# nianticlabs/mickey

Measured on AMD Instinct MI355X. Metric: image pairs/sec (540x720), higher is better.
Workload: dtype bf16

## Files before the change

### mickey_amd/csrc/mk_attention.hip

```cpp
#include <type_traits>

#include "mk_common.hpp"

namespace mk {
void launch_attn_f32(const float* q, const float* k, const float* vt, float* out, int ldo, int nimg, int heads, int ntok,
                     int ntok_pad, hipStream_t st);
}

namespace {
using namespace mk;

constexpr int KV_TILE_BYTES = 64 * 64 * 2;
constexpr float ATT_REBASE_SUM = 4096.0f;

struct AttnBlock {
  int qblk, head, img;
};
__device__ __forceinline__ AttnBlock attn_block() {
  const int lin = blockIdx.x + gridDim.x * (blockIdx.y + gridDim.y * blockIdx.z);
  const int r = xcd_remap(lin, gridDim.x * gridDim.y * gridDim.z);
  const int hg = r / gridDim.x;
  return AttnBlock{r - hg * (int)gridDim.x, hg % (int)gridDim.y, hg / (int)gridDim.y};
}

template <typename T, int QB>
__global__ __launch_bounds__(256, 2) void attn_fwd_kernel(const T* __restrict__ q, const T* __restrict__ k,
                                                          const T* __restrict__ vt, T* __restrict__ out, int ldo, int heads,
                                                          int ntok, int ntok_pad) {
  using V8 = typename Lp<T>::V8;
  using V4 = typename Lp<T>::V4;
  __shared__ __attribute__((aligned(16))) char smem[4 * KV_TILE_BYTES];

  const int lane = threadIdx.x & 63;
  const int wave = __builtin_amdgcn_readfirstlane(threadIdx.x >> 6);
  const AttnBlock ab = attn_block();
  const int head = ab.head, img = ab.img;
  const long long hb = (long long)img * heads + head;
  const T* Qh = q + hb * ntok_pad * 64;
  const T* Kh = k + hb * ntok_pad * 64;
  const T* Vh = vt + hb * 64 * ntok_pad;
  const int q0 = ab.qblk * (128 * QB) + wave * (32 * QB);
  const int j = lane & 31, hi = lane >> 5;
  const bool wave_has_queries = q0 < ntok;

  V8 qf[QB][4];
#pragma unroll
  for (int qb = 0; qb < QB; ++qb) {
    int qrow = q0 + qb * 32 + j;
    qrow = qrow < ntok_pad ? qrow : ntok_pad - 1;
#pragma unroll
    for (int ks = 0; ks < 4; ++ks) qf[qb][ks] = *(const V8*)(Qh + (long long)qrow * 64 + ks * 16 + hi * 8);
  }

  const int srow = lane >> 3, sp = lane & 7;
  auto stage = [&](int buf, int kt) {
    char* sK = smem + buf * 2 * KV_TILE_BYTES;
    char* sV = sK + KV_TILE_BYTES;
#pragma unroll
    for (int t = 0; t < 2; ++t) {
      const int ii = wave * 2 + t;
      const int r = ii * 8 + srow;
      glds16(Kh + (long long)(kt * 64 + r) * 64 + swz8(r, sp) * 8, sK + ii * 1024);
      glds16(Vh + (long long)r * ntok_pad + kt * 64 + swz8(r, sp) * 8, sV + ii * 1024);
    }
  };

  f32x16 o[QB][2];
  float m_run[QB], l_run[QB];
#pragma unroll
  for (int qb = 0; qb < QB; ++qb) {
#pragma unroll
    for (int i = 0; i < 16; ++i) o[qb][0][i] = o[qb][1][i] = 0.f;
    m_run[qb] = -1e30f;
    l_run[qb] = 0.f;
  }

  const int nkt = (ntok + 63) >> 6;
  stage(0, 0);
  auto kv_tile = [&](const int kt, auto last_tag) {
    constexpr bool LAST = decltype(last_tag)::value;
    asm volatile("s_waitcnt vmcnt(0)" ::: "memory");
    __syncthreads();
    if (!LAST) stage((kt + 1) & 1, kt + 1);
    if (!wave_has_queries) return;
    const char* sK = smem + (kt & 1) * 2 * KV_TILE_BYTES;
    const char* sV = sK + KV_TILE_BYTES;

    f32x16 s[QB][2];
#pragma unroll
    for (int kb = 0; kb < 2; ++kb) {
#pragma unroll
      for (int qb = 0; qb < QB; ++qb)
#pragma unroll
        for (int i = 0; i < 16; ++i) s[qb][kb][i] = 0.f;
      const int row = kb * 32 + j;
#pragma unroll
      for (int ks = 0; ks < 4; ++ks) {
        const V8 kf = *(const V8*)(sK + row * 128 + swz8(row, ks * 2 + hi) * 16);
#pragma unroll
        for (int qb = 0; qb < QB; ++qb) s[qb][kb] = Lp<T>::mma32(kf, qf[qb][ks], s[qb][kb]);
      }
    }
    V8 pf[QB][4];
#pragma unroll
    for (int qb = 0; qb < QB; ++qb) {
      if (LAST && (ntok & 63)) {
#pragma unroll
        for (int kb = 0; kb < 2; ++kb)
#pragma unroll
          for (int r = 0; r < 16; ++r) {
            const int key = kt * 64 + kb * 32 + (r & 3) + 8 * (r >> 2) + 4 * hi;
            if (key >= ntok) s[qb][kb][r] = -1e30f;
          }
      }
      float t8[8];
#pragma unroll
      for (int r = 0; r < 8; ++r)
        t8[r] = fmaxf(fmaxf(s[qb][0][r], s[qb][0][r + 8]), fmaxf(s[qb][1][r], s[qb][1][r + 8]));
      float mx = fmaxf(fmaxf(fmaxf(t8[0], t8[1]), t8[2]), fmaxf(fmaxf(t8[3], t8[4]), t8[5]));
      mx = fmaxf(fmaxf(mx, t8[6]), t8[7]);
      mx = fmaxf(mx, __shfl_xor(mx, 32, 64));
      const float m_new = fmaxf(m_run[qb], mx);
      const bool grew = m_new > m_run[qb];
      float rs4[4] = {0.f, 0.f, 0.f, 0.f};
#pragma unroll
      for (int kb = 0; kb < 2; ++kb)
#pragma unroll
        for (int r = 0; r < 16; ++r) {
          const float pv = __builtin_amdgcn_exp2f(s[qb][kb][r] - m_new);
          s[qb][kb][r] = pv;
          rs4[r & 3] += pv;
        }
      const float rs = (rs4[0] + rs4[1]) + (rs4[2] + rs4[3]);
      if (__any(grew)) {
        const float alpha = __builtin_amdgcn_exp2f(m_run[qb] - m_new);
        l_run[qb] *= alpha;
#pragma unroll
        for (int i = 0; i < 16; ++i) {
          o[qb][0][i] *= alpha;
          o[qb][1][i] *= alpha;
        }
      }
      m_run[qb] = m_new;
      l_run[qb] += rs;
#pragma unroll
      for (int s4 = 0; s4 < 4; ++s4)
#pragma unroll
        for (int e = 0; e < 8; ++e) pf[qb][s4][e] = (T)s[qb][s4 >> 1][(s4 & 1) * 8 + e];
    }
#pragma unroll
    for (int dt = 0; dt < 2; ++dt) {
      const int row = dt * 32 + j;
#pragma unroll
      for (int s4 = 0; s4 < 4; ++s4) {
        const V8 vf = *(const V8*)(sV + row * 128 + swz8(row, s4 * 2 + hi) * 16);
#pragma unroll
        for (int qb = 0; qb < QB; ++qb) o[qb][dt] = Lp<T>::mma32(vf, pf[qb][s4], o[qb][dt]);
      }
    }
  };
  for (int kt = 0; kt < nkt - 1; ++kt) kv_tile(kt, std::false_type{});
  kv_tile(nkt - 1, std::true_type{});

#pragma unroll
  for (int qb = 0; qb < QB; ++qb) {
    const float l_tot = l_run[qb] + __shfl_xor(l_run[qb], 32, 64);
    const float inv = 1.0f / l_tot;
    const int qi = q0 + qb * 32 + j;
    if (qi < ntok) {
      T* orow = out + ((long long)img * ntok + qi) * ldo + head * 64;
#pragma unroll
      for (int dt = 0; dt < 2; ++dt)
#pragma unroll
        for (int r4 = 0; r4 < 4; ++r4) {
          V4 w;
#pragma unroll
          for (int e = 0; e < 4; ++e) w[e] = (T)(o[qb][dt][r4 * 4 + e] * inv);
          *(V4*)(orow + dt * 32 + r4 * 8 + hi * 4) = w;
        }
    }
  }
}

template <typename T, int QB>
__device__ __forceinline__ void attn_fold_wave(const T* __restrict__ Qh, const T* __restrict__ Kh, const T* __restrict__ Vh,
                                               T* __restrict__ out, int ldo, int img, int head, int ntok, int ntok_pad, char* smem,
                                               int lane, int wave, int q0) {
  using V8 = typename Lp<T>::V8;
  using V4 = typename Lp<T>::V4;
  const int j = lane & 31, hi = lane >> 5;
  const bool wave_has_queries = q0 < ntok;

  V8 qf[QB][4];
#pragma unroll
  for (int qb = 0; qb < QB; ++qb) {
    int qrow = q0 + qb * 32 + j;
    qrow = qrow < ntok_pad ? qrow : ntok_pad - 1;
#pragma unroll
    for (int ks = 0; ks < 4; ++ks) qf[qb][ks] = *(const V8*)(Qh + (long long)qrow * 64 + ks * 16 + hi * 8);
  }
  const int srow = lane >> 3, sp = lane & 7;
  auto stage = [&](int buf, int kt) {
    char* sK = smem + buf * 2 * KV_TILE_BYTES;
    char* sV = sK + KV_TILE_BYTES;
#pragma unroll
    for (int t = 0; t < 2; ++t) {
      const int ii = wave * 2 + t;
      const int r = ii * 8 + srow;
      glds16(Kh + (long long)(kt * 64 + r) * 64 + swz8(r, sp) * 8, sK + ii * 1024);
      glds16(Vh + (long long)r * ntok_pad + kt * 64 + swz8(r, sp) * 8, sV + ii * 1024);
    }
  };

  f32x16 o[QB][2], negm[QB];
  float m_run[QB], l_run[QB];
#pragma unroll
  for (int qb = 0; qb < QB; ++qb) {
#pragma unroll
    for (int i = 0; i < 16; ++i) {
      o[qb][0][i] = o[qb][1][i] = 0.f;
      negm[qb][i] = 0.f;
    }
    m_run[qb] = l_run[qb] = 0.f;
  }
  bool first = true;

  const int nkt = (ntok + 63) >> 6;
  stage(0, 0);
  auto kv_tile = [&](const int kt, auto last_tag) {
    constexpr bool LAST = decltype(last_tag)::value;
    asm volatile("s_waitcnt vmcnt(0)" ::: "memory");
    __syncthreads();
    if (!LAST) stage((kt + 1) & 1, kt + 1);
    if (!wave_has_queries) return;
    const char* sK = smem + (kt & 1) * 2 * KV_TILE_BYTES;
    const char* sV = sK + KV_TILE_BYTES;

    f32x16 s[QB][2];
    const bool half_tile = LAST && (ntok & 63) != 0 && (ntok & 63) <= 32;
#pragma unroll
    for (int kb = 0; kb < 2; ++kb) {
      if (LAST && kb == 1 && half_tile) {
#pragma unroll
        for (int qb = 0; qb < QB; ++qb)
#pragma unroll
          for (int r = 0; r < 16; ++r) s[qb][1][r] = -1e30f;
        continue;
      }
      const int row = kb * 32 + j;
#pragma unroll
      for (int ks = 0; ks < 4; ++ks) {
        const V8 kf = *(const V8*)(sK + row * 128 + swz8(row, ks * 2 + hi) * 16);
#pragma unroll
        for (int qb = 0; qb < QB; ++qb) s[qb][kb] = Lp<T>::mma32(kf, qf[qb][ks], ks == 0 ? negm[qb] : s[qb][kb]);
      }
    }
    V8 pf[QB][4];
#pragma unroll
    for (int qb = 0; qb < QB; ++qb) {
      if (LAST && (ntok & 63)) {
#pragma unroll
        for (int kb = 0; kb < 2; ++kb)
#pragma unroll
          for (int r = 0; r < 16; ++r) {
            const int key = kt * 64 + kb * 32 + (r & 3) + 8 * (r >> 2) + 4 * hi;
            if (key >= ntok) s[qb][kb][r] = -1e30f;
          }
      }
      auto exp_sum = [&]() {
        float rs4[4] = {0.f, 0.f, 0.f, 0.f};
#pragma unroll
        for (int s4 = 0; s4 < 4; ++s4)
#pragma unroll
          for (int e = 0; e < 8; ++e) {
            const float pv = __builtin_amdgcn_exp2f(s[qb][s4 >> 1][(s4 & 1) * 8 + e]);
            pf[qb][s4][e] = (T)pv;
            rs4[e & 3] += pv;
          }
        return (rs4[0] + rs4[1]) + (rs4[2] + rs4[3]);
      };
      float rs = 0.f;
      bool rebase = first;
      if (!first) {
        rs = exp_sum();
        rebase = __any(!(rs <= ATT_REBASE_SUM));
      }
      if (rebase) {
        float t8[8];
#pragma unroll
        for (int r = 0; r < 8; ++r) t8[r] = fmaxf(fmaxf(s[qb][0][r], s[qb][0][r + 8]), fmaxf(s[qb][1][r], s[qb][1][r + 8]));
        float mx = fmaxf(fmaxf(fmaxf(t8[0], t8[1]), t8[2]), fmaxf(fmaxf(t8[3], t8[4]), t8[5]));
        mx = fmaxf(fmaxf(mx, t8[6]), t8[7]);
        mx = fmaxf(mx, __shfl_xor(mx, 32, 64));
        const float shift = first ? mx : fmaxf(mx, 0.f);
        const float alpha = first ? 1.0f : __builtin_amdgcn_exp2f(-shift);
#pragma unroll
        for (int i = 0; i < 16; ++i) {
          o[qb][0][i] *= alpha;
          o[qb][1][i] *= alpha;
          s[qb][0][i] -= shift;
          s[qb][1][i] -= shift;
        }
        l_run[qb] *= alpha;
        m_run[qb] += shift;
#pragma unroll
        for (int i = 0; i < 16; ++i) negm[qb][i] = -m_run[qb];
        rs = exp_sum();
      }
      l_run[qb] += rs;
    }
    first = false;
#pragma unroll
    for (int dt = 0; dt < 2; ++dt) {
      const int row = dt * 32 + j;
#pragma unroll
      for (int s4 = 0; s4 < 4; ++s4) {
        if (LAST && s4 >= 2 && half_tile) break;
        const V8 vf = *(const V8*)(sV + row * 128 + swz8(row, s4 * 2 + hi) * 16);
#pragma unroll
        for (int qb = 0; qb < QB; ++qb) o[qb][dt] = Lp<T>::mma32(vf, pf[qb][s4], o[qb][dt]);
      }
    }
  };
  for (int kt = 0; kt < nkt - 1; ++kt) kv_tile(kt, std::false_type{});
  kv_tile(nkt - 1, std::true_type{});

#pragma unroll
  for (int qb = 0; qb < QB; ++qb) {
    const float inv = 1.0f / (l_run[qb] + __shfl_xor(l_run[qb], 32, 64));
    const int qi = q0 + qb * 32 + j;
    if (qi < ntok) {
      T* orow = out + ((long long)img * ntok + qi) * ldo + head * 64;
#pragma unroll
      for (int dt = 0; dt < 2; ++dt)
#pragma unroll
        for (int r4 = 0; r4 < 4; ++r4) {
          V4 w;
#pragma unroll
          for (int e = 0; e < 4; ++e) w[e] = (T)(o[qb][dt][r4 * 4 + e] * inv);
          *(V4*)(orow + dt * 32 + r4 * 8 + hi * 4) = w;
        }
    }
  }
}

template <typename T, int QB, bool TAIL1 = true>
__global__ __launch_bounds__(256, QB == 2 ? 2 : 3) void attn_fwd_fold_kernel(const T* __restrict__ q, const T* __restrict__ k,
                                                                              const T* __restrict__ vt, T* __restrict__ out,
                                                                              int ldo, int heads, int ntok, int ntok_pad) {
  __shared__ __attribute__((aligned(16))) char smem[4 * KV_TILE_BYTES];
  const int lane = threadIdx.x & 63;
  const int wave = __builtin_amdgcn_readfirstlane(threadIdx.x >> 6);
  const AttnBlock ab = attn_block();
  const int head = ab.head, img = ab.img;
  const long long hb = (long long)img * heads + head;
  const T* Qh = q + hb * ntok_pad * 64;
  const T* Kh = k + hb * ntok_pad * 64;
  const T* Vh = vt + hb * 64 * ntok_pad;
  const int q0 = ab.qblk * (128 * QB) + wave * (32 * QB);
  if constexpr (QB == 2 && TAIL1) {
    if (q0 < ntok && q0 + 32 >= ntok) {
      attn_fold_wave<T, 1>(Qh, Kh, Vh, out, ldo, img, head, ntok, ntok_pad, smem, lane, wave, q0);
      return;
    }
  }
  attn_fold_wave<T, QB>(Qh, Kh, Vh, out, ldo, img, head, ntok, ntok_pad, smem, lane, wave, q0);
}

template <typename T, int QB>
__global__ __launch_bounds__(256, QB == 2 ? 2 : 3) void attn_fwd_fold16_kernel(const T* __restrict__ q, const T* __restrict__ k,
                                                                                const T* __restrict__ vt, T* __restrict__ out,
                                                                                int ldo, int heads, int ntok, int ntok_pad) {
  using V8 = typename Lp<T>::V8;
  using V4 = typename Lp<T>::V4;
  __shared__ __attribute__((aligned(16))) char smem[4 * KV_TILE_BYTES];

  const int lane = threadIdx.x & 63;
  const int wave = __builtin_amdgcn_readfirstlane(threadIdx.x >> 6);
  const AttnBlock ab = attn_block();
  const int head = ab.head, img = ab.img;
  const long long hb = (long long)img * heads + head;
  const T* Qh = q + hb * ntok_pad * 64;
  const T* Kh = k + hb * ntok_pad * 64;
  const T* Vh = vt + hb * 64 * ntok_pad;
  const int q0 = ab.qblk * (128 * QB) + wave * (32 * QB);
  const int n = lane & 15, g = lane >> 4;
  const bool wave_has_queries = q0 < ntok;

  V8 qf[QB][2][2];
#pragma unroll
  for (int qb = 0; qb < QB; ++qb)
#pragma unroll
    for (int nb = 0; nb < 2; ++nb) {
      int qrow = q0 + qb * 32 + nb * 16 + n;
      qrow = qrow < ntok_pad ? qrow : ntok_pad - 1;
#pragma unroll
      for (int ks = 0; ks < 2; ++ks) qf[qb][nb][ks] = *(const V8*)(Qh + (long long)qrow * 64 + ks * 32 + g * 8);
    }
  const int srow = lane >> 3, sp = lane & 7;
  auto stage = [&](int buf, int kt) {
    char* sK = smem + buf * 2 * KV_TILE_BYTES;
    char* sV = sK + KV_TILE_BYTES;
#pragma unroll
    for (int t = 0; t < 2; ++t) {
      const int ii = wave * 2 + t;
      const int r = ii * 8 + srow;
      glds16(Kh + (long long)(kt * 64 + r) * 64 + swz8(r, sp) * 8, sK + ii * 1024);
      glds16(Vh + (long long)r * ntok_pad + kt * 64 + swz8(r, sp) * 8, sV + ii * 1024);
    }
  };

  f32x4 o[QB][2][4], negm[QB][2];
  float m_run[QB][2], l_run[QB][2];
#pragma unroll
  for (int qb = 0; qb < QB; ++qb)
#pragma unroll
    for (int nb = 0; nb < 2; ++nb) {
#pragma unroll
      for (int db = 0; db < 4; ++db) o[qb][nb][db] = f32x4{0.f, 0.f, 0.f, 0.f};
      negm[qb][nb] = f32x4{0.f, 0.f, 0.f, 0.f};
      m_run[qb][nb] = l_run[qb][nb] = 0.f;
    }
  bool first = true;
  const int pq = ((g & 1) << 1) | (g >> 1);

  const int nkt = (ntok + 63) >> 6;
  stage(0, 0);
  auto kv_tile = [&](const int kt, auto last_tag) {
    constexpr bool LAST = decltype(last_tag)::value;
    asm volatile("s_waitcnt vmcnt(0)" ::: "memory");
    __syncthreads();
    if (!LAST) stage((kt + 1) & 1, kt + 1);
    if (!wave_has_queries) return;
    const char* sK = smem + (kt & 1) * 2 * KV_TILE_BYTES;
    const char* sV = sK + KV_TILE_BYTES;

    f32x4 s[QB][2][4];
#pragma unroll
    for (int ks = 0; ks < 2; ++ks) {
#pragma unroll
      for (int kb = 0; kb < 4; ++kb) {
        const int row = kb * 16 + n;
        const V8 kf = *(const V8*)(sK + row * 128 + swz8(row, ks * 4 + g) * 16);
#pragma unroll
        for (int qb = 0; qb < QB; ++qb)
#pragma unroll
          for (int nb = 0; nb < 2; ++nb)
            s[qb][nb][kb] = Lp<T>::mma16(kf, qf[qb][nb][ks], ks == 0 ? negm[qb][nb] : s[qb][nb][kb]);
      }
    }
    V8 pf[QB][2][2];
#pragma unroll
    for (int qb = 0; qb < QB; ++qb)
#pragma unroll
      for (int nb = 0; nb < 2; ++nb) {
        if (LAST && (ntok & 63)) {
#pragma unroll
          for (int kb = 0; kb < 4; ++kb)
#pragma unroll
            for (int r = 0; r < 4; ++r)
              if (kt * 64 + kb * 16 + 4 * g + r >= ntok) s[qb][nb][kb][r] = -1e30f;
        }
        auto exp_sum = [&]() {
          float rs4[4] = {0.f, 0.f, 0.f, 0.f};
#pragma unroll
          for (int kb = 0; kb < 4; ++kb)
#pragma unroll
            for (int r = 0; r < 4; ++r) {
              const float pv = __builtin_amdgcn_exp2f(s[qb][nb][kb][r]);
              pf[qb][nb][kb >> 1][(kb & 1) * 4 + r] = (T)pv;
              rs4[r] += pv;
            }
          return (rs4[0] + rs4[1]) + (rs4[2] + rs4[3]);
        };
        float rs = 0.f;
        bool rebase = first;
        if (!first) {
          rs = exp_sum();
          rebase = __any(!(rs <= ATT_REBASE_SUM));
        }
        if (rebase) {
          float t4[4];
#pragma unroll
          for (int r = 0; r < 4; ++r) t4[r] = fmaxf(fmaxf(s[qb][nb][0][r], s[qb][nb][1][r]), fmaxf(s[qb][nb][2][r], s[qb][nb][3][r]));
          float mx = fmaxf(fmaxf(t4[0], t4[1]), fmaxf(t4[2], t4[3]));
          mx = fmaxf(mx, __shfl_xor(mx, 16, 64));
          mx = fmaxf(mx, __shfl_xor(mx, 32, 64));
          const float shift = first ? mx : fmaxf(mx, 0.f);
          const float alpha = first ? 1.0f : __builtin_amdgcn_exp2f(-shift);
#pragma unroll
          for (int b4 = 0; b4 < 4; ++b4)
#pragma unroll
            for (int i = 0; i < 4; ++i) {
              o[qb][nb][b4][i] *= alpha;
              s[qb][nb][b4][i] -= shift;
// ... 108 lines not shown
```

### mickey_amd/csrc/mk_gemm_common.hpp

```cpp
#pragma once
#include "mk_common.hpp"

namespace mk {
namespace gemm {

constexpr int BK = 64;
template <typename T> constexpr int EPC = 16 / (int)sizeof(T);
template <typename T> constexpr int KT = 128 / (int)sizeof(T);

enum AMode { A_DENSE = 0, A_CONV3 = 1 };

struct GemmParams {
  const void* A;
  const void* A2;
  const void* W;
  int M, N, K, lda, ldw;
  long long strideA_g, strideA2_g, strideW_g;
  int H, Wd, C1, C2;
  int bord_out;
  unsigned pl1[2], pl2[2];
  int npass;
  float acc_scale;
  void* out_lo;
  float plane_scale;
  int* sat_flag;
  int epi;
  int act;
  const float* bias;
  const float* gamma;
  long long strideBias_g;
  float* out_f32;
  void* out_lp;
  int ldc;
  long long strideOut_g;
  const void* resid_lp;
  long long strideResid_g;
  void* q;
  void* k;
  void* vt;
  int ntok, ntok_pad, heads;
  float qscale;
  const float* pos;
  int npatch;
  void* xh;
  void* xl;
  int ldxs;
  float* stats_out;
  int nslot_out;
  const float* ln_stats;
  const float* ln_colsum;
  int ln_nslot;
  float ln_eps;
  float* ln_shift_out;
  const float* ln_shift_in;
};

__device__ __forceinline__ void quad_stats(const f32x4& x, float& s, float& q) {
  s = x[0];
  s += x[1];
  s += x[2];
  s += x[3];
  q = __builtin_fmaf(x[0], x[0], 0.0f);
  q = __builtin_fmaf(x[1], x[1], q);
  q = __builtin_fmaf(x[2], x[2], q);
  q = __builtin_fmaf(x[3], x[3], q);
}

__device__ __forceinline__ float row16_sum(float v) {
#define MK_DPP_ADD(ctrl) v += __builtin_bit_cast(float, __builtin_amdgcn_update_dpp(0, __builtin_bit_cast(int, v), ctrl, 0xf, 0xf, true))
  MK_DPP_ADD(0xB1);
  MK_DPP_ADD(0x4E);
  MK_DPP_ADD(0x141);
  MK_DPP_ADD(0x140);
#undef MK_DPP_ADD
  return v;
}

typedef __attribute__((ext_vector_type(4))) unsigned u32x4;
struct LnRowLoads16 {
  u32x4 v[4];
  __device__ __forceinline__ void issue(const GemmParams& p, int m0, int tid) {
    const int wave = tid >> 6, lane = tid & 63;
    const long long last = (long long)p.M * 128 - 16;
#pragma unroll
    for (int j = 0; j < 4; ++j) {
      long long off = ((long long)(m0 + wave * 32 + j * 8) * 128) + lane * 16;
      off = off < last ? off : last;
      const char* a = (const char*)p.ln_stats + off;
      asm volatile("global_load_dwordx4 %0, %1, off" : "=v"(v[j]) : "v"(a) : "memory");
    }
  }
  template <int YOUNGER>
  __device__ __forceinline__ void finish(const GemmParams& p, int tid, float2* prm, int m0 = 0, bool publish = false) {
    asm volatile("s_waitcnt vmcnt(%4)" : "+v"(v[0]), "+v"(v[1]), "+v"(v[2]), "+v"(v[3]) : "n"(YOUNGER) : "memory");
    const int wave = tid >> 6, lane = tid & 63;
#pragma unroll
    for (int j = 0; j < 4; ++j) {
      const f32x4 f = __builtin_bit_cast(f32x4, v[j]);
      float s = f[0] + f[2], q = f[1] + f[3];
#define MK_DPP_ADD(x, ctrl) x += __builtin_bit_cast(float, __builtin_amdgcn_update_dpp(0, __builtin_bit_cast(int, x), ctrl, 0xf, 0xf, true))
      MK_DPP_ADD(s, 0xB1);  MK_DPP_ADD(q, 0xB1);
      MK_DPP_ADD(s, 0x4E);  MK_DPP_ADD(q, 0x4E);
      MK_DPP_ADD(s, 0x141); MK_DPP_ADD(q, 0x141);
#undef MK_DPP_ADD
      const double mean = (double)s * (1.0 / 1024.0);
      double var = (double)q * (1.0 / 1024.0) - mean * mean;
      var = var > 0.0 ? var : 0.0;
      const float rstd = 1.0f / sqrtf((float)var + p.ln_eps);
      if ((lane & 7) == 0) {
        const int r = wave * 32 + j * 8 + (lane >> 3);
        prm[r] = make_float2(rstd, -(float)mean * rstd);
        if (publish && m0 + r < p.M) p.ln_shift_out[m0 + r] = (float)mean;
      }
    }
  }
};

struct LnRowDma16 {
  template <int J0>
  __device__ __forceinline__ static void issue(const GemmParams& p, int m0, int wave, int lane, char* stage_lds) {
    const long long last = (long long)p.M * 128 - 16;
#pragma unroll
    for (int j = J0; j < J0 + 2; ++j) {
      const long long base = (long long)(m0 + wave * 32 + j * 8) * 128;
      long long off = base + lane * 16;
      off = off < last ? off : last;
      glds16_sv((const char*)p.ln_stats, (unsigned)off, stage_lds + (wave * 2 + (j - J0)) * 1024);
    }
  }
  template <int J0>
  __device__ __forceinline__ static void finish(const GemmParams& p, int wave, int lane, float2* prm, const char* stage_lds, int m0,
                                                bool publish) {
#pragma unroll
    for (int j = J0; j < J0 + 2; ++j) {
      const f32x4 f = *(const f32x4*)(stage_lds + (wave * 2 + (j - J0)) * 1024 + lane * 16);
      float s = f[0] + f[2], q = f[1] + f[3];
#define MK_DPP_ADD(x, ctrl) x += __builtin_bit_cast(float, __builtin_amdgcn_update_dpp(0, __builtin_bit_cast(int, x), ctrl, 0xf, 0xf, true))
      MK_DPP_ADD(s, 0xB1);  MK_DPP_ADD(q, 0xB1);
      MK_DPP_ADD(s, 0x4E);  MK_DPP_ADD(q, 0x4E);
      MK_DPP_ADD(s, 0x141); MK_DPP_ADD(q, 0x141);
#undef MK_DPP_ADD
      const double mean = (double)s * (1.0 / 1024.0);
      double var = (double)q * (1.0 / 1024.0) - mean * mean;
      var = var > 0.0 ? var : 0.0;
      const float rstd = 1.0f / sqrtf((float)var + p.ln_eps);
      if ((lane & 7) == 0) {
        const int r = wave * 32 + j * 8 + (lane >> 3);
        prm[r] = make_float2(rstd, -(float)mean * rstd);
        if (publish && m0 + r < p.M) p.ln_shift_out[m0 + r] = (float)mean;
      }
    }
  }
};

struct ShiftLoad {
  float v;
  __device__ __forceinline__ void issue(const GemmParams& p, int m0, int tid, int BM) {
    v = 0.f;
    if (p.ln_shift_in && tid < BM) {
      int m = m0 + tid;
      m = m < p.M ? m : p.M - 1;
      const float* a = p.ln_shift_in + m;
      asm volatile("global_load_dword %0, %1, off" : "=v"(v) : "v"(a) : "memory");
    }
  }
  template <int YOUNGER>
  __device__ __forceinline__ void finish(int tid, int BM, float* shl) {
    if constexpr (YOUNGER >= 0)
      asm volatile("s_waitcnt vmcnt(%1)" : "+v"(v) : "n"(YOUNGER) : "memory");
    else
      asm volatile("" : "+v"(v) : : "memory");
    if (tid < BM) shl[tid] = v;
  }
};

template <int BM, int NT>
__device__ __forceinline__ void ln_params_to_lds(const GemmParams& p, int m0, int tid, float2* prm, bool publish = false) {
  static_assert(NT == 2 * BM, "two threads per row");
  const int r = tid >> 1, h = tid & 1;
  int m = m0 + r;
  m = m < p.M ? m : p.M - 1;
  const float2* st = (const float2*)p.ln_stats + (long long)m * p.ln_nslot;
  float s, q;
  if (p.ln_nslot <= 16) {
    float2 v[8];
#pragma unroll
    for (int j = 0; j < 8; ++j) v[j] = 8 * h + j < p.ln_nslot ? st[8 * h + j] : make_float2(0.f, 0.f);
    const float s01 = v[0].x + v[1].x, s23 = v[2].x + v[3].x, s45 = v[4].x + v[5].x, s67 = v[6].x + v[7].x;
    const float q01 = v[0].y + v[1].y, q23 = v[2].y + v[3].y, q45 = v[4].y + v[5].y, q67 = v[6].y + v[7].y;
    s = (s01 + s23) + (s45 + s67);
    q = (q01 + q23) + (q45 + q67);
  } else {
    const int per = (p.ln_nslot + 1) >> 1;
    const int lo = h * per, hi = min(p.ln_nslot, lo + per);
    s = q = 0.f;
    for (int i0 = lo; i0 < hi; i0 += 8) {
      float2 v[8];
#pragma unroll
      for (int j = 0; j < 8; ++j) v[j] = i0 + j < hi ? st[i0 + j] : make_float2(0.f, 0.f);
#pragma unroll
      for (int j = 0; j < 8; ++j) {
        s += v[j].x;
        q += v[j].y;
      }
    }
  }
  s += __shfl_xor(s, 1, 64);
  q += __shfl_xor(q, 1, 64);
  const double invn = 1.0 / (64.0 * p.ln_nslot);
  const double mean = (double)s * invn;
  double var = (double)q * invn - mean * mean;
  var = var > 0.0 ? var : 0.0;
  const float rstd = 1.0f / sqrtf((float)var + p.ln_eps);
  if (h == 0) {
    prm[r] = make_float2(rstd, -(float)mean * rstd);
    if (publish && m0 + r < p.M) p.ln_shift_out[m0 + r] = (float)mean;
  }
}

template <typename T>
__device__ __forceinline__ T to_lp(float v) { return (T)v; }

template <typename T>
__device__ __forceinline__ f32x4 unpack4(uint2 u);
template <>
__device__ __forceinline__ f32x4 unpack4<__bf16>(uint2 u) {
  return f32x4{__builtin_bit_cast(float, u.x << 16), __builtin_bit_cast(float, u.x & 0xffff0000u),
               __builtin_bit_cast(float, u.y << 16), __builtin_bit_cast(float, u.y & 0xffff0000u)};
}
template <>
// ... 132 lines not shown
#pragma unroll
          for (int e = 0; e < 4; ++e) r[e] = (float)h[e] + (float)l[e];
          r += gm * v;
          r -= shv;
          v = r;
        } else {
          v += *(const f32x4*)(p.pos + (long long)tok1 * p.N + n);
        }
        if (fin) {
          *(f32x4*)(p.out_f32 + xrow * p.ldc + n) = v;
          continue;
        }
        V4 oh, ol;
#pragma unroll
        for (int e = 0; e < 4; ++e) {
          oh[e] = to_lp<T>(v[e]);
          ol[e] = to_lp<T>(v[e] - (float)oh[e]);
        }
        quad_stats(v, s4[ni], q4[ni]);
        *(V4*)ph = oh;
        *(V4*)pl = ol;
      }
#pragma unroll
      for (int ni = 0; ni < 4; ++ni) {
        s4[ni] += __shfl_xor(s4[ni], 16, 64);
        q4[ni] += __shfl_xor(q4[ni], 16, 64);
        s4[ni] += __shfl_xor(s4[ni], 32, 64);
        q4[ni] += __shfl_xor(q4[ni], 32, 64);
      }
      const float ssum = (s4[0] + s4[1]) + (s4[2] + s4[3]), qsum = (q4[0] + q4[1]) + (q4[2] + q4[3]);
      if (!fin && fg == 0 && mok && n0 + wn * 64 < p.N)
        ((float2*)p.stats_out)[xrow * p.nslot_out + ((n0 + wn * 64) >> 6)] = make_float2(ssum, qsum);
      continue;
    }
    if (m >= p.M) continue;
    float2 prm = make_float2(1.f, 0.f);
    if (LN) prm = lnp[wm * (WMF * 16) + mi * 16 + fr];
    int img = 0, tok = 0;
    if (EPI == MK_EPI_QKV) {
      img = m / p.ntok;
      tok = m - img * p.ntok;
    } else if (EPI == MK_EPI_PATCH) {
      img = m / p.npatch;
      tok = m - img * p.npatch;
    }
    const long long brow = (EPI == MK_EPI_STORE && p.H > 0) ? bordered_row(m, p.H, p.Wd) : (long long)m;
#pragma unroll
    for (int ni = 0; ni < 4; ++ni) {
      const int n = nb + ni * 16;
      if (n >= p.N) continue;
      f32x4 v = acc[mi][ni];
      if (EPI == MK_EPI_STORE && p.npass > 1) {
        const float sc = p.acc_scale;
#pragma unroll
        for (int e = 0; e < 4; ++e) v[e] *= sc;
      }
      if (LN) v = v * prm.x + (cs[ni] * prm.y + bv[ni]);
      else if (HAS_BIAS) v += bv[ni];
      if (EPI == MK_EPI_STORE) {
        if (p.resid_lp) {
          const V4 r = *(const V4*)((const T*)p.resid_lp + (long long)g * p.strideResid_g + brow * p.ldc + n);
#pragma unroll
          for (int e = 0; e < 4; ++e) v[e] += (float)r[e];
        }
        if (ACT == MK_ACT_RELU) {
#pragma unroll
          for (int e = 0; e < 4; ++e) v[e] = fmaxf(v[e], 0.f);
        } else if (ACT == MK_ACT_GELU) {
          v = gelu_erf4(v);
        }
        if (p.out_lo) {
          const float ps = p.plane_scale;
          f16x4 oh, ol;
#pragma unroll
          for (int e = 0; e < 4; ++e) {
            const float sv = sat16(v[e] * ps, p.sat_flag);
            oh[e] = (_Float16)sv;
            ol[e] = (_Float16)(sv - (float)oh[e]);
          }
          const long long o = (long long)g * p.strideOut_g + (p.bord_out ? brow : (long long)m) * p.ldc + n;
          *(f16x4*)((_Float16*)p.out_lp + o) = oh;
          *(f16x4*)((_Float16*)p.out_lo + o) = ol;
        } else if (p.out_f32) {
          *(f32x4*)(p.out_f32 + (long long)g * p.strideOut_g + (p.bord_out ? brow : (long long)m) * p.ldc + n) = v;
        } else {
          V4 o;
#pragma unroll
          for (int e = 0; e < 4; ++e) o[e] = to_lp<T>(v[e]);
          *(V4*)((T*)p.out_lp + (long long)g * p.strideOut_g + (p.bord_out ? brow : (long long)m) * p.ldc + n) = o;
        }
      } else if (EPI == MK_EPI_LS_RESIDUAL) {
        float* x = p.out_f32 + (long long)m * p.ldc + n;
        const f32x4 gm = *(const f32x4*)(p.gamma + n);
        f32x4 r = *(const f32x4*)x;
        r += gm * v;
        *(f32x4*)x = r;
      } else if (EPI == MK_EPI_PATCH) {
        const f32x4 pe = *(const f32x4*)(p.pos + (long long)(1 + tok) * p.N + n);
        *(f32x4*)(p.out_f32 + ((long long)img * (p.npatch + 1) + 1 + tok) * p.ldc + n) = v + pe;
      } else {
        const int D = p.heads * 64;
        const int which = n / D;
        const int rem = n - which * D;
        const int head = rem >> 6, d = rem & 63;
        const long long hb = (long long)img * p.heads + head;
        if (which == 2) {
          T* dst = (T*)p.vt + (hb * 64 + d) * p.ntok_pad + vperm(tok);
#pragma unroll
          for (int e = 0; e < 4; ++e) dst[(long long)e * p.ntok_pad] = to_lp<T>(v[e]);
        } else {
          if (which == 0) { const float qs = p.qscale; _Pragma("unroll") for (int e = 0; e < 4; ++e) v[e] *= qs; }
          V4 o;
#pragma unroll
          for (int e = 0; e < 4; ++e) o[e] = to_lp<T>(v[e]);
          T* base = (T*)(which == 0 ? p.q : p.k);
          *(V4*)(base + (hb * p.ntok_pad + tok) * 64 + d) = o;
        }
      }
    }
  }
}

template <typename T, int WMF>
__device__ __forceinline__ void epilogue(const GemmParams& p, f32x4 (&acc)[WMF][4], int m0, int n0, int wm, int wn, int lane,
                                         int g, const float2* lnp = nullptr) {
  if (p.xh) {
    if (p.epi == MK_EPI_PATCH) epilogue_impl<T, WMF, MK_EPI_PATCH, MK_ACT_NONE, true, false, true>(p, acc, m0, n0, wm, wn, lane, g);
    else epilogue_impl<T, WMF, MK_EPI_LS_RESIDUAL, MK_ACT_NONE, true, false, true>(p, acc, m0, n0, wm, wn, lane, g);
    return;
  }
  if (p.ln_stats) {
    if (p.epi == MK_EPI_QKV) epilogue_impl<T, WMF, MK_EPI_QKV, MK_ACT_NONE, true, true>(p, acc, m0, n0, wm, wn, lane, g, lnp);
    else if (p.act == MK_ACT_GELU) epilogue_impl<T, WMF, MK_EPI_STORE, MK_ACT_GELU, true, true>(p, acc, m0, n0, wm, wn, lane, g, lnp);
    else epilogue_impl<T, WMF, MK_EPI_STORE, MK_ACT_NONE, true, true>(p, acc, m0, n0, wm, wn, lane, g, lnp);
    return;
  }
  switch (p.epi) {
    case MK_EPI_LS_RESIDUAL: epilogue_impl<T, WMF, MK_EPI_LS_RESIDUAL, MK_ACT_NONE, true>(p, acc, m0, n0, wm, wn, lane, g); break;
    case MK_EPI_QKV: epilogue_impl<T, WMF, MK_EPI_QKV, MK_ACT_NONE, true>(p, acc, m0, n0, wm, wn, lane, g); break;
    case MK_EPI_PATCH: epilogue_impl<T, WMF, MK_EPI_PATCH, MK_ACT_NONE, true>(p, acc, m0, n0, wm, wn, lane, g); break;
    default:
      if (!p.bias) {
        if (p.act == MK_ACT_RELU) epilogue_impl<T, WMF, MK_EPI_STORE, MK_ACT_RELU, false>(p, acc, m0, n0, wm, wn, lane, g);
        else if (p.act == MK_ACT_GELU) epilogue_impl<T, WMF, MK_EPI_STORE, MK_ACT_GELU, false>(p, acc, m0, n0, wm, wn, lane, g);
        else epilogue_impl<T, WMF, MK_EPI_STORE, MK_ACT_NONE, false>(p, acc, m0, n0, wm, wn, lane, g);
      } else {
        if (p.act == MK_ACT_RELU) epilogue_impl<T, WMF, MK_EPI_STORE, MK_ACT_RELU, true>(p, acc, m0, n0, wm, wn, lane, g);
        else if (p.act == MK_ACT_GELU) epilogue_impl<T, WMF, MK_EPI_STORE, MK_ACT_GELU, true>(p, acc, m0, n0, wm, wn, lane, g);
        else epilogue_impl<T, WMF, MK_EPI_STORE, MK_ACT_NONE, true>(p, acc, m0, n0, wm, wn, lane, g);
      }
  }
}

template <typename T, int EPI, int ACT, bool HAS_BIAS, bool LN = false, bool SPLIT = false, bool FIN = false, bool CONV = false>
__device__ __forceinline__ void epilogue_lds_impl(const GemmParams& p, f32x4 (&acc)[8][4], char* wl0, char* wl1, int m0, int n0, int wm,
                                                  int wn, int lane, int g, const float2* lnp = nullptr) {
  using V4 = typename Lp<T>::V4;
  using V8 = typename Lp<T>::V8;
  const int fr = lane & 15, fg = lane >> 4;
  const float* bias = HAS_BIAS ? p.bias + (long long)g * p.strideBias_g : nullptr;
  const int nw = n0 + wn * 64;
  const int mw = m0 + wm * 128;
  int img0 = 0, tok0 = 0;
  if (EPI == MK_EPI_QKV) {
    img0 = mw / p.ntok;
    tok0 = mw - img0 * p.ntok;
  }
  auto img_tok = [&](int r, int& img, int& tok) {
    if (p.ntok >= 128) {
      const int t = tok0 + r;
      const bool wrap = t >= p.ntok;
      img = img0 + (wrap ? 1 : 0);
      tok = wrap ? t - p.ntok : t;
    } else {
      const int m = mw + r;
      img = m / p.ntok;
      tok = m - img * p.ntok;
    }
  };
  f32x4 bv[4], cs[4];
#pragma unroll
  for (int ni = 0; ni < 4; ++ni) {
    const int n = nw + fg * 4 + ni * 16;
    bv[ni] = (HAS_BIAS && n < p.N) ? *(const f32x4*)(bias + n) : f32x4{0.f, 0.f, 0.f, 0.f};
    cs[ni] = (LN && n < p.N) ? *(const f32x4*)(p.ln_colsum + n) : f32x4{0.f, 0.f, 0.f, 0.f};
  }
  float2 prm[8];
#pragma unroll
  for (int mi = 0; mi < 8; ++mi) prm[mi] = LN ? lnp[wm * 128 + mi * 16 + fr] : make_float2(1.f, 0.f);
  const bool lp_out = EPI == MK_EPI_QKV || (EPI == MK_EPI_STORE && !p.out_f32 && !p.out_lo);
  if (lp_out) {
    int which = 0, head = 0;
    if (EPI == MK_EPI_QKV) {
      const int D = p.heads * 64;
      which = nw / D;
      head = (nw - which * D) >> 6;
      if (which == 2) {
#pragma unroll
        for (int mi = 0; mi < 8; ++mi) {
          const int m = mw + mi * 16 + fr;
          if (m >= p.M) continue;
          int img, tok;
          img_tok(mi * 16 + fr, img, tok);
          const long long hb = (long long)img * p.heads + head;
#pragma unroll
          for (int ni = 0; ni < 4; ++ni) {
            const f32x4 v = LN ? acc[mi][ni] * prm[mi].x + (cs[ni] * prm[mi].y + bv[ni]) : acc[mi][ni] + bv[ni];
            T* dst = (T*)p.vt + (hb * 64 + ni * 16 + fg * 4) * p.ntok_pad + vperm(tok);
#pragma unroll
            for (int e = 0; e < 4; ++e) dst[(long long)e * p.ntok_pad] = to_lp<T>(v[e]);
          }
        }
        return;
      }
    }
    const int rr = lane >> 3, c = lane & 7;
    const int n = nw + c * 8;
    const bool bord = CONV && p.bord_out;
    BorderedRow bw;
    if (bord) bw.init(mw + rr, p.H, p.Wd);
#pragma unroll
    for (int h = 0; h < 2; ++h) {
#pragma unroll
      for (int mq = 0; mq < 4; ++mq) {
        const int mi = h * 4 + mq;
        const int r = mi * 16 + fr;
        char* wrow = (mq < 2 ? wl0 : wl1) + ((mq & 1) * 16 + fr) * 128;
        const long long rrow = (CONV && p.resid_lp) ? bordered_row(min(mw + r, p.M - 1), p.H, p.Wd) : 0;
#pragma unroll
        for (int ni = 0; ni < 4; ++ni) {
          f32x4 v = acc[mi][ni];
          if (LN) v = v * prm[mi].x + (cs[ni] * prm[mi].y + bv[ni]);
          else if (HAS_BIAS) v += bv[ni];
          if (EPI == MK_EPI_QKV) {
            if (which == 0) { const float qs = p.qscale; _Pragma("unroll") for (int e = 0; e < 4; ++e) v[e] *= qs; }
          } else {
            if (CONV && p.resid_lp) {
              const int m = mw + r, n2 = nw + fg * 4 + ni * 16;
              if (m < p.M && n2 < p.N) {
                const V4 rs = *(const V4*)((const T*)p.resid_lp + (long long)g * p.strideResid_g + rrow * p.ldc + n2);
#pragma unroll
                for (int e = 0; e < 4; ++e) v[e] += (float)rs[e];
              }
            }
            if (ACT == MK_ACT_RELU) {
#pragma unroll
              for (int e = 0; e < 4; ++e) v[e] = fmaxf(v[e], 0.f);
            } else if (ACT == MK_ACT_GELU) {
              v = gelu_erf4(v);
            }
          }
          V4 o;
#pragma unroll
          for (int e = 0; e < 4; ++e) o[e] = to_lp<T>(v[e]);
          const int cc = ni * 2 + (fg >> 1);
          *(V4*)(wrow + ((cc ^ (fr & 7)) << 4) + (fg & 1) * 8) = o;
        }
      }
#pragma unroll
      for (int i8 = 0; i8 < 8; ++i8) {
        const int it = h * 8 + i8;
        const int r = it * 8 + rr;
        const int m = mw + r;
        const V8 val = *(const V8*)((i8 < 4 ? wl0 : wl1) + ((i8 & 3) * 8 + rr) * 128 + ((c ^ (rr & 7)) << 4));
        const int extra = bord ? bw.extra : 0;
        if (bord) bw.step(8, p.H, p.Wd);
        if (m >= p.M || n >= p.N) continue;
        T* dst;
        if (EPI == MK_EPI_QKV) {
          int img, tok;
          img_tok(r, img, tok);
          dst = (T*)(which == 0 ? p.q : p.k) + (((long long)img * p.heads + head) * p.ntok_pad + tok) * 64 + c * 8;
        } else {
          dst = (T*)p.out_lp + (long long)g * p.strideOut_g + ((long long)m + extra) * p.ldc + n;
        }
        if (n + 8 <= p.N) {
          *(V8*)dst = val;
        } else {
          V4 lo;
#pragma unroll
          for (int e = 0; e < 4; ++e) lo[e] = val[e];
          *(V4*)dst = lo;
        }
      }
    }
  } else {
    const int rr = lane >> 4, c = lane & 15;
    const int n = nw + c * 4;
    f32x4 gm = f32x4{0.f, 0.f, 0.f, 0.f};
    if (EPI == MK_EPI_LS_RESIDUAL && n < p.N) gm = *(const f32x4*)(p.gamma + n);
    f32x4 bvd = f32x4{0.f, 0.f, 0.f, 0.f};
    if (SPLIT && HAS_BIAS && n < p.N) bvd = *(const f32x4*)(bias + n);
    f32x4 xr[2][SPLIT ? 1 : 16];
    uint2 xh[2][SPLIT ? 16 : 1], xl[2][SPLIT ? 16 : 1];
    const unsigned lane_off = (unsigned)rr * (unsigned)p.ldxs + (unsigned)n;
    unsigned lane_off_st = lane_off;
    asm volatile("" : "+v"(lane_off_st));
    auto plane_row = [&](void* plane, int half, int it) -> T* {
      return (T*)plane + (long long)(mw + half * 64 + it * 4) * p.ldxs;
    };
    __amdgpu_buffer_rsrc_t rs_h, rs_l;
    unsigned voff_b = 0;
    if constexpr (SPLIT && EPI == MK_EPI_LS_RESIDUAL && sizeof(T) == 2) {
      rs_h = __builtin_amdgcn_make_buffer_rsrc(p.xh, 0, 0x7fffffff, 0x00020000);
      rs_l = __builtin_amdgcn_make_buffer_rsrc(p.xl, 0, 0x7fffffff, 0x00020000);
      voff_b = lane_off * 2u;
    }
    auto soff_b = [&](int half, int it) -> unsigned {
      return (unsigned)(mw + half * 64 + it * 4) * (unsigned)p.ldxs * 2u;
    };
    typedef unsigned u32x2_t __attribute__((ext_vector_type(2)));
    auto preload = [&](int half, int it0 = 0, int it1 = 16) {
      if (EPI != MK_EPI_LS_RESIDUAL) return;
#pragma unroll
      for (int it = 0; it < 16; ++it) {
        if (it < it0 || it >= it1) continue;
        const int m = mw + half * 64 + it * 4 + rr;
        const bool ok = SPLIT || (m < p.M && n < p.N);
        if constexpr (SPLIT && EPI == MK_EPI_LS_RESIDUAL && sizeof(T) == 2) {
          const u32x2_t a = __builtin_amdgcn_raw_buffer_load_b64(rs_h, voff_b, soff_b(half, it), 0);
          const u32x2_t b = __builtin_amdgcn_raw_buffer_load_b64(rs_l, voff_b, soff_b(half, it), 0);
          xh[half][it] = uint2{a[0], a[1]};
          xl[half][it] = uint2{b[0], b[1]};
        } else if (SPLIT) {
          xh[half][it] = ok ? *(const uint2*)(plane_row(p.xh, half, it) + lane_off) : uint2{0u, 0u};
          xl[half][it] = ok ? *(const uint2*)(plane_row(p.xl, half, it) + lane_off) : uint2{0u, 0u};
        } else {
          xr[half][it] = ok ? *(const f32x4*)(p.out_f32 + (long long)m * p.ldc + n) : f32x4{0.f, 0.f, 0.f, 0.f};
        }
      }
    };
    auto stageq = [&](int half, int sub) {
#pragma unroll
      for (int m2 = 0; m2 < 2; ++m2) {
        const int mi = sub * 2 + m2;
        const int r = mi * 16 + fr;
        char* wrow = (m2 == 0 ? wl0 : wl1) + fr * 256;
        const long long rrow = (CONV && p.resid_lp) ? bordered_row(min(mw + half * 64 + r, p.M - 1), p.H, p.Wd) : 0;
#pragma unroll
        for (int ni = 0; ni < 4; ++ni) {
          f32x4 v = acc[half * 4 + mi][ni];
          if (EPI == MK_EPI_STORE && p.npass > 1) {
            const float sc = p.acc_scale;
#pragma unroll
            for (int e = 0; e < 4; ++e) v[e] *= sc;
          }
          if (HAS_BIAS && !SPLIT) v += bv[ni];
          if (EPI == MK_EPI_STORE) {
            if (CONV && p.resid_lp) {
              const int m = mw + half * 64 + r, nn = nw + fg * 4 + ni * 16;
              if (m < p.M && nn < p.N) {
                const V4 rs = *(const V4*)((const T*)p.resid_lp + (long long)g * p.strideResid_g + rrow * p.ldc + nn);
#pragma unroll
                for (int e = 0; e < 4; ++e) v[e] += (float)rs[e];
              }
            }
            if (ACT == MK_ACT_RELU) {
#pragma unroll
              for (int e = 0; e < 4; ++e) v[e] = fmaxf(v[e], 0.f);
            } else if (ACT == MK_ACT_GELU) {
              v = gelu_erf4(v);
            }
          }
          const int cw = ni * 4 + fg;
          *(f32x4*)(wrow + ((cw ^ fr) << 4)) = v;
        }
      }
    };
    constexpr bool fin = FIN;
    auto emit_row = [&](long long xrow, T* dh, T* dl, f32x4 x, bool ok, unsigned soff = 0xffffffffu) {
      float ssum = 0.f, qsum = 0.f;
      if (ok) {
        const uint2 oh = pack4<T>(x);
        const uint2 ol = pack4<T>(x - unpack4<T>(oh));
        quad_stats(x, ssum, qsum);
        if constexpr (SPLIT && EPI == MK_EPI_LS_RESIDUAL && sizeof(T) == 2) {
          __builtin_amdgcn_raw_buffer_store_b64(u32x2_t{oh.x, oh.y}, rs_h, voff_b, soff, 0);
          __builtin_amdgcn_raw_buffer_store_b64(u32x2_t{ol.x, ol.y}, rs_l, voff_b, soff, 0);
        } else {
          *(uint2*)dh = oh;
          *(uint2*)dl = ol;
        }
      }
      ssum = row16_sum(ssum);
      qsum = row16_sum(qsum);
      if (ok && c == 0) ((float2*)p.stats_out)[xrow * p.nslot_out + (nw >> 6)] = make_float2(ssum, qsum);
    };
    auto drain = [&](int half, int it0 = 0, int it1 = 16) {
      const bool bordf = CONV && p.bord_out;
      BorderedRow bwf;
      if (bordf) bwf.init(mw + half * 64 + it0 * 4 + rr, p.H, p.Wd);
#pragma unroll
      for (int it = 0; it < 16; ++it) {
        if (it < it0 || it >= it1) continue;
        const int r = it * 4 + rr;
        const int m = mw + half * 64 + r;
        const int extraf = bordf ? bwf.extra : 0;
        if (bordf) bwf.step(4, p.H, p.Wd);
        f32x4 val = *(const f32x4*)(((it & 4) ? wl1 : wl0) + ((it & 3) * 4 + rr) * 256 + ((c ^ ((it & 3) * 4 + rr)) << 4));
        if (SPLIT) val += bvd;
        const bool ok = SPLIT || (m < p.M && n < p.N);
        if (!ok) continue;
        if (EPI == MK_EPI_LS_RESIDUAL) {
          f32x4 x;
          if (SPLIT) {
            x = unpack4<T>(xh[half][it]) + unpack4<T>(xl[half][it]);
          } else {
            x = xr[half][it];
          }
          x += gm * val;
          if (SPLIT) x -= ((const float*)lnp)[wm * 128 + half * 64 + r];
          if (!SPLIT || fin) {
            if (ok) *(f32x4*)(p.out_f32 + (long long)m * p.ldc + n) = x;
          } else {
            if constexpr (sizeof(T) == 2) emit_row(m, nullptr, nullptr, x, ok, soff_b(half, it));
            else emit_row(m, plane_row(p.xh, half, it) + lane_off_st, plane_row(p.xl, half, it) + lane_off_st, x, ok);
          }
        } else if (EPI == MK_EPI_PATCH) {
          const int mc = ok ? m : 0;
          const int img = mc / p.npatch, tok = mc - img * p.npatch;
          const long long xrow = (long long)img * (p.npatch + 1) + 1 + tok;
          f32x4 x = val;
          if (ok) x += *(const f32x4*)(p.pos + (long long)(1 + tok) * p.N + n);
          if (SPLIT) emit_row(xrow, (T*)p.xh + xrow * p.ldxs + n, (T*)p.xl + xrow * p.ldxs + n, x, ok);
          else if (ok) *(f32x4*)(p.out_f32 + xrow * p.ldc + n) = x;
        } else if (EPI == MK_EPI_STORE && p.out_lo) {
          const float ps = p.plane_scale;
          f16x4 oh, ol;
#pragma unroll
          for (int e = 0; e < 4; ++e) {
            const float sv = sat16(val[e] * ps, p.sat_flag);
            oh[e] = (_Float16)sv;
            ol[e] = (_Float16)(sv - (float)oh[e]);
          }
          const long long o = (long long)g * p.strideOut_g + ((long long)m + extraf) * p.ldc + n;
          *(f16x4*)((_Float16*)p.out_lp + o) = oh;
          *(f16x4*)((_Float16*)p.out_lo + o) = ol;
        } else {
// ... 99 lines not shown
```

Before: 276.7.

## Widen attention output stores and add 16-byte split-plane residual epilogue

The attention output path now converts each row to 8-byte packets and, when the output pointer and stride are 16-byte aligned, uses permlane32 swaps so each lane writes full 16-byte vectors instead of 8-byte ones. Separately, a specialized epilogue for the split hi/lo residual plus layer-scale GEMM path uses 8 lanes per row with 16-byte buffer loads and stores and an 8-lane DPP row reduction for LN stats. It interleaves plane preloads with LDS staging. Both changes aim to cut memory transaction count, at the cost of extra cross-lane shuffles and more live registers.

```diff
diff --git a/mickey_amd/csrc/mk_attention.hip b/mickey_amd/csrc/mk_attention.hip
--- a/mickey_amd/csrc/mk_attention.hip
+++ b/mickey_amd/csrc/mk_attention.hip
@@ -21,6 +21,40 @@
   const int r = xcd_remap(lin, gridDim.x * gridDim.y * gridDim.z);
   const int hg = r / gridDim.x;
   return AttnBlock{r - hg * (int)gridDim.x, hg % (int)gridDim.y, hg / (int)gridDim.y};
+}
+
+template <typename T>
+__device__ __forceinline__ void store_o_row(T* __restrict__ orow, bool valid, bool wide, const f32x16 (&o)[2], float inv, int hi) {
+  using V4 = typename Lp<T>::V4;
+  typedef unsigned u32x2_t __attribute__((ext_vector_type(2)));
+  typedef unsigned u32x4_t __attribute__((ext_vector_type(4)));
+  u32x2_t w[8];
+#pragma unroll
+  for (int g = 0; g < 8; ++g) {
+    V4 v;
+#pragma unroll
+    for (int e = 0; e < 4; ++e) v[e] = (T)(o[g >> 2][(g & 3) * 4 + e] * inv);
+    w[g] = __builtin_bit_cast(u32x2_t, v);
+  }
+  if (wide) {
+    u32x4_t w16[4];
+#pragma unroll
+    for (int g = 0; g < 8; g += 2) {
+      const auto x = __builtin_amdgcn_permlane32_swap(w[g][0], w[g + 1][0], false, false);
+      const auto y = __builtin_amdgcn_permlane32_swap(w[g][1], w[g + 1][1], false, false);
+      w16[g >> 1] = u32x4_t{x[0], y[0], x[1], y[1]};
+    }
+    if (valid) {
+#pragma unroll
+      for (int p = 0; p < 4; ++p) *(u32x4_t*)(orow + p * 16 + hi * 8) = w16[p];
+    }
+  } else if (valid) {
+#pragma unroll
+    for (int g = 0; g < 8; ++g) *(u32x2_t*)(orow + g * 8 + hi * 4) = w[g];
+  }
+}
+__device__ __forceinline__ bool o_rows_16b_aligned(const void* out, int ldo) {
+  return ((reinterpret_cast<unsigned long long>(out) | ((unsigned long long)ldo * 2)) & 15) == 0;
 }
 
 template <typename T, int QB>
@@ -167,18 +201,7 @@
     const float l_tot = l_run[qb] + __shfl_xor(l_run[qb], 32, 64);
     const float inv = 1.0f / l_tot;
     const int qi = q0 + qb * 32 + j;
-    if (qi < ntok) {
-      T* orow = out + ((long long)img * ntok + qi) * ldo + head * 64;
-#pragma unroll
-      for (int dt = 0; dt < 2; ++dt)
-#pragma unroll
-        for (int r4 = 0; r4 < 4; ++r4) {
-          V4 w;
-#pragma unroll
-          for (int e = 0; e < 4; ++e) w[e] = (T)(o[qb][dt][r4 * 4 + e] * inv);
-          *(V4*)(orow + dt * 32 + r4 * 8 + hi * 4) = w;
-        }
-    }
+    store_o_row<T>(out + ((long long)img * ntok + qi) * ldo + head * 64, qi < ntok, o_rows_16b_aligned(out, ldo), o[qb], inv, hi);
   }
 }
 
@@ -329,18 +352,7 @@
   for (int qb = 0; qb < QB; ++qb) {
     const float inv = 1.0f / (l_run[qb] + __shfl_xor(l_run[qb], 32, 64));
     const int qi = q0 + qb * 32 + j;
-    if (qi < ntok) {
-      T* orow = out + ((long long)img * ntok + qi) * ldo + head * 64;
-#pragma unroll
-      for (int dt = 0; dt < 2; ++dt)
-#pragma unroll
-        for (int r4 = 0; r4 < 4; ++r4) {
-          V4 w;
-#pragma unroll
-          for (int e = 0; e < 4; ++e) w[e] = (T)(o[qb][dt][r4 * 4 + e] * inv);
-          *(V4*)(orow + dt * 32 + r4 * 8 + hi * 4) = w;
-        }
-    }
+    store_o_row<T>(out + ((long long)img * ntok + qi) * ldo + head * 64, qi < ntok, o_rows_16b_aligned(out, ldo), o[qb], inv, hi);
   }
 }
 
diff --git a/mickey_amd/csrc/mk_gemm_common.hpp b/mickey_amd/csrc/mk_gemm_common.hpp
--- a/mickey_amd/csrc/mk_gemm_common.hpp
+++ b/mickey_amd/csrc/mk_gemm_common.hpp
@@ -76,6 +76,15 @@
   return v;
 }
 
+__device__ __forceinline__ float row8_sum(float v) {
+#define MK_DPP_ADD(ctrl) v += __builtin_bit_cast(float, __builtin_amdgcn_update_dpp(0, __builtin_bit_cast(int, v), ctrl, 0xf, 0xf, true))
+  MK_DPP_ADD(0xB1);
+  MK_DPP_ADD(0x4E);
+  MK_DPP_ADD(0x141);
+#undef MK_DPP_ADD
+  return v;
+}
+
 typedef __attribute__((ext_vector_type(4))) unsigned u32x4;
 struct LnRowLoads16 {
   u32x4 v[4];
@@ -514,6 +523,114 @@
   }
 }
 
+template <typename T, bool FIN>
+__device__ __forceinline__ void epilogue_lds_split16(const GemmParams& p, f32x4 (&acc)[8][4], char* wl0, char* wl1, int m0, int n0,
+                                                     int wm, int wn, int lane, int g, const float2* lnp) {
+  static_assert(sizeof(T) == 2, "16-bit planes");
+  typedef unsigned u32x4_t __attribute__((ext_vector_type(4)));
+  const int fr = lane & 15, fg = lane >> 4;
+  const int rr = lane >> 3, l = lane & 7;
+  const int nw = n0 + wn * 64;
+  const int mw = m0 + wm * 128;
+  const int n = nw + l * 8;
+  const float* bias = p.bias + (long long)g * p.strideBias_g;
+  f32x4 gm[2], bvd[2];
+#pragma unroll
+  for (int k = 0; k < 2; ++k) {
+    gm[k] = *(const f32x4*)(p.gamma + n + 4 * k);
+    bvd[k] = *(const f32x4*)(bias + n + 4 * k);
+  }
+  const __amdgpu_buffer_rsrc_t rs_h = __builtin_amdgcn_make_buffer_rsrc(p.xh, 0, 0x7fffffff, 0x00020000);
+  const __amdgpu_buffer_rsrc_t rs_l = __builtin_amdgcn_make_buffer_rsrc(p.xl, 0, 0x7fffffff, 0x00020000);
+  const unsigned voff_b = ((unsigned)rr * (unsigned)p.ldxs + (unsigned)n) * 2u;
+  auto soff_b = [&](int half, int it) -> unsigned { return (unsigned)(mw + half * 64 + it * 8) * (unsigned)p.ldxs * 2u; };
+  u32x4_t xh[2][8], xl[2][8];
+  auto preload = [&](int half, int it0, int it1) {
+#pragma unroll
+    for (int it = 0; it < 8; ++it) {
+      if (it < it0 || it >= it1) continue;
+      xh[half][it] = __builtin_amdgcn_raw_buffer_load_b128(rs_h, voff_b, soff_b(half, it), 0);
+      xl[half][it] = __builtin_amdgcn_raw_buffer_load_b128(rs_l, voff_b, soff_b(half, it), 0);
+    }
+  };
+  auto stageq = [&](int half, int sub) {
+#pragma unroll
+    for (int m2 = 0; m2 < 2; ++m2) {
+      char* wrow = (m2 == 0 ? wl0 : wl1) + fr * 256;
+#pragma unroll
+      for (int ni = 0; ni < 4; ++ni) *(f32x4*)(wrow + (((ni * 4 + fg) ^ fr) << 4)) = acc[half * 4 + sub * 2 + m2][ni];
+    }
+  };
+  float keep_s = 0.f, keep_q = 0.f;
+  auto drain = [&](int half, int it0, int it1) {
+#pragma unroll
+    for (int it = 0; it < 8; ++it) {
+      if (it < it0 || it >= it1) continue;
+      const int r = it * 8 + rr;
+      const int sr = (it & 1) * 8 + rr;
+      const char* srow = ((it & 2) ? wl1 : wl0) + sr * 256;
+      const float shift = ((const float*)lnp)[wm * 128 + half * 64 + r];
+      const uint2 h2[2] = {uint2{xh[half][it][0], xh[half][it][1]}, uint2{xh[half][it][2], xh[half][it][3]}};
+      const uint2 l2[2] = {uint2{xl[half][it][0], xl[half][it][1]}, uint2{xl[half][it][2], xl[half][it][3]}};
+      f32x4 x[2];
+#pragma unroll
+      for (int k = 0; k < 2; ++k) {
+        f32x4 val = *(const f32x4*)(srow + (((2 * l + k) ^ sr) << 4));
+        val += bvd[k];
+        x[k] = unpack4<T>(h2[k]) + unpack4<T>(l2[k]);
+        x[k] += gm[k] * val;
+        x[k] -= shift;
+      }
+      if (FIN) {
+        float* dst = p.out_f32 + (long long)(mw + half * 64 + r) * p.ldc + n;
+        *(f32x4*)dst = x[0];
+        *(f32x4*)(dst + 4) = x[1];
+      } else {
+        uint2 oh[2], ol[2];
+        float s2[2], q2[2];
+#pragma unroll
+        for (int k = 0; k < 2; ++k) {
+          oh[k] = pack4<T>(x[k]);
+          ol[k] = pack4<T>(x[k] - unpack4<T>(oh[k]));
+          quad_stats(x[k], s2[k], q2[k]);
+        }
+        __builtin_amdgcn_raw_buffer_store_b128(u32x4_t{oh[0].x, oh[0].y, oh[1].x, oh[1].y}, rs_h, voff_b, soff_b(half, it), 0);
+        __builtin_amdgcn_raw_buffer_store_b128(u32x4_t{ol[0].x, ol[0].y, ol[1].x, ol[1].y}, rs_l, voff_b, soff_b(half, it), 0);
+        const float ssum = row8_sum(s2[0] + s2[1]);
+        const float qsum = row8_sum(q2[0] + q2[1]);
+        keep_s = l == it ? ssum : keep_s;
+        keep_q = l == it ? qsum : keep_q;
+      }
+    }
+    if (!FIN && it1 == 8)
+      ((float2*)p.stats_out)[(long long)(mw + half * 64 + l * 8 + rr) * p.nslot_out + (nw >> 6)] = make_float2(keep_s, keep_q);
+  };
+  if (!FIN) {
+    preload(0, 0, 8);
+    stageq(0, 0);
+    drain(0, 0, 4);
+    preload(1, 0, 4);
+    stageq(0, 1);
+    drain(0, 4, 8);
+    preload(1, 4, 8);
+    stageq(1, 0);
+    drain(1, 0, 4);
+    stageq(1, 1);
+    drain(1, 4, 8);
+  } else {
+    preload(0, 0, 8);
+    stageq(0, 0);
+    drain(0, 0, 4);
+    stageq(0, 1);
+    preload(1, 0, 8);
+    drain(0, 4, 8);
+    stageq(1, 0);
+    drain(1, 0, 4);
+    stageq(1, 1);
+    drain(1, 4, 8);
+  }
+}
+
 template <typename T, int EPI, int ACT, bool HAS_BIAS, bool LN = false, bool SPLIT = false, bool FIN = false, bool CONV = false>
 __device__ __forceinline__ void epilogue_lds_impl(const GemmParams& p, f32x4 (&acc)[8][4], char* wl0, char* wl1, int m0, int n0, int wm,
                                                   int wn, int lane, int g, const float2* lnp = nullptr) {
@@ -646,6 +763,8 @@
         }
       }
     }
+  } else if constexpr (SPLIT && EPI == MK_EPI_LS_RESIDUAL && sizeof(T) == 2 && HAS_BIAS && !CONV) {
+    epilogue_lds_split16<T, FIN>(p, acc, wl0, wl1, m0, n0, wm, wn, lane, g, lnp);
   } else {
     const int rr = lane >> 4, c = lane & 15;
     const int n = nw + c * 4;
```

Result: no change. 278.7 (median of 6 runs) (+0.7%).
